# konstantineder/montecarlo-risk-engine

Measured on AMD Instinct MI355X. Metric: path-steps/sec at 1M paths x 250 steps; PV/CVA rel-error vs CPU ref, higher is better.
Workload: dtype f64

## Files before the change

montecarlo-risk-engine_amd/csrc/kf_common.h:

```cpp
#pragma once
#include <cstddef>
#include "mcx_device.h"



struct FAtom {
    int32_t reg, pad;
    double a, d, b, c0, c1;
};
struct FTerm { double w; FAtom atom; };
struct FEvent {
    int32_t kind, flags;
    int32_t term_begin, term_end;
    int32_t coeff_off, row;
    int32_t ns, sidx;
    int32_t init_state, pad;
    double strike, sign;
    double aux[4];
    FAtom num, x;
};
struct FMetricOp {
    int32_t ns, m;
    int32_t rec_profile;
    int32_t has_cva;
    double threshold;
    FAtom surv, cond;
};

struct ChunkHeader { int32_t n_ev, n_mop, n_terms, bytes; };

struct FastDate {
    int32_t valid, flags;
    int32_t ni_reg, lin_reg, n_exp, x_reg, coeff_off0, coeff_off1, rec_profile, s_reg, c_reg, pad;
    int32_t t_reg[4];
    double x_a, x_d;
    double c_a, c_b, c_c0, c_c1;
    double m_b, m_c0, m_n1, m_s1;
    double ni_c0, ni_c1;
    double k0, k1;
    double t_w[4], t_c0[4], t_c1[4];
    double thr;
    double s_b, s_c0, s_c1;
    int32_t ex_n, ex_term_off, ex_coeff_off, ex_x_reg, ex_lin_reg, ex_pad;
    double ex_k0, ex_k1, ex_strike, ex_sign, ex_x_a, ex_x_d;
    double op_strike, op_sign;
    double ex_p_lo, ex_p_hi, ex_p_ms, ex_p_ih;
    int32_t ex_p_off, ex_p_blk, ex_p_reg, ex_p_pad;
};
struct FastDateHot {
    int32_t valid, flags;
    int32_t ni_reg, lin_reg, n_exp, x_reg, coeff_off0, coeff_off1, rec_profile, s_reg, c_reg, pad;
    int32_t t_reg[4];
    double x_a, x_d;
    double c_a, c_b, c_c0, c_c1;
    double m_b, m_c0, m_n1, m_s1;
};
static_assert(sizeof(FastDateHot) == 144 && offsetof(FastDate, ni_c0) == sizeof(FastDateHot), "FastDateHot must mirror the head of FastDate");
struct LeanTerm { double w, c0, c1; int32_t reg, pad; };

struct FusedArgs {
    K1Args k1;
    const FastDate* __restrict__ fast;
    const LeanTerm* __restrict__ lterms;
    const double* __restrict__ vcoef;
    const unsigned char* __restrict__ prog;
    const int32_t* __restrict__ date_off;
    const int32_t* __restrict__ date_row;
    const double* __restrict__ coeffs;
    double* __restrict__ cfs;
    double* __restrict__ expo;
    double* __restrict__ partials;
    int64_t ld_out;
    int32_t n_dates, n_basis, n_ns, n_rec, n_expo_rows, n_stateful, chunk_cap, pad;
    int32_t rec_pv[MCX_FUSED_MAX_NS];
    int32_t rec_cva[MCX_FUSED_MAX_NS];
    double lgd[MCX_FUSED_MAX_NS];
    int32_t init_state[MCX_FUSED_MAX_STATEFUL];
};

__device__ __forceinline__ void chan_merge(double& N, double& mean, double& M2, double n, double m, double q)
{
    if (n <= 0.0) return;
    if (N == 0.0) { N = n; mean = m; M2 = q; return; }
    const double delta = m - mean, tot = N + n;
    mean += delta * n / tot;
    M2 += q + delta * delta * N * n / tot;
    N = tot;
}

#define RFL(x) __builtin_amdgcn_readfirstlane(x)

template <int NREG>
__device__ __forceinline__ double f_atom(const FAtom& a, const double (&reg)[NREG])
{
    const int r = RFL(a.reg), fl = RFL(a.pad);
    const double x = r >= 0 ? reg[r] : 0.0;
    double v = (fl & 2) ? fma(a.d, x, a.a) : 0.0;
    if (fl & 1) v = fma(a.b, mcx_exp(fma(a.c1, x, a.c0)), v);
    return v;
}

__device__ __forceinline__ double f_poly_uniform(const double* __restrict__ coeffs, int off_vgpr, int K, double x)
{
    const double* __restrict__ c = coeffs + __builtin_amdgcn_readfirstlane(off_vgpr);
    double v = 0.0, xp = 1.0;
#pragma unroll 1
    for (int k = 0; k < K; ++k) { v = fma(ldk(c + k), xp, v); xp *= x; }
    return v;
}

__device__ __forceinline__ double f_poly(const double* __restrict__ c, int K, double x)
{
    double v = 0.0, xp = 1.0;
#pragma unroll 1
    for (int k = 0; k < K; ++k) { v = fma(c[k], xp, v); xp *= x; }
    return v;
}

__device__ __forceinline__ void f_record(double v, bool live, int rec, int n_rec, bool first_tile, double* __restrict__ lds)
{
    if (first_tile) {
        __syncthreads();
        if (threadIdx.x == 0) lds[rec] = v;
        __syncthreads();
    }
    const double c = lds[rec];
    const double d = live ? v - c : 0.0;
    const double s1 = wave_sum(d), s2 = wave_sum(d * d);
    if ((threadIdx.x & 63) == 0) {
        double* acc = lds + n_rec + ((threadIdx.x >> 6) * n_rec + rec) * 2;
        acc[0] += s1;
        acc[1] += s2;
    }
}

template <int NREG>
__device__ __forceinline__ double f_regsel(int r, const double (&reg)[NREG])
{
    return r >= 0 ? reg[r] : 0.0;
}


int mcx_launch_kf_lean(const FusedArgs& a, const mcx_sim_desc& sd, int n_cu, bool inject, bool simulate, hipStream_t s);
```

montecarlo-risk-engine_amd/csrc/kf_fused.hip:

```cpp
#include "kf_common.h"

#include <algorithm>
#include <type_traits>
#include <cmath>
#include <cstdlib>

namespace {

template <int NSLOT, int SIG, int NNS, bool STORE, bool ALL_FAST>
__device__ __forceinline__ bool kf_fast_date(const FusedArgs& a, int t, int64_t i, bool live, bool first_tile, double* __restrict__ lds,
                                             const double (&reg)[2 * NSLOT], double (&cfs)[NNS], double (&cva)[NNS])
{
    constexpr int NREG = 2 * NSLOT;
    if (NNS != 1) return false;
    if (!ALL_FAST && ldk(&a.fast[t].valid) != 1) return false;
    const FastDate* __restrict__ fp = a.fast + t;
#define FD(x) ldk(&fp->x)
    const K1Args& k = a.k1;
    if (STORE && k.paths && live) sim_store_state<NSLOT, SIG>(k, t, i, reg);
    const int flags = FD(flags);
    const double inv = (flags & 16) ? FD(ni_c0) : mcx_exp(fma(FD(ni_c1), f_regsel<NREG>(FD(ni_reg), reg), FD(ni_c0)));
    if (flags & 1) {
        double val = fma(FD(k1), f_regsel<NREG>(FD(lin_reg), reg), FD(k0));
        const int n_exp = FD(n_exp);
// ... 271 lines not shown
                on_date(t, std::integral_constant<bool, false>());
                next_t = t + 1;
            }
        }
        (void)next_t;
        for (int w = 0; w < a.n_ns; ++w) {
            double cv = cfs[0], cc = cva[0];
#pragma unroll
            for (int q = 1; q < NNS; ++q) { cv = (w == q) ? cfs[q] : cv; cc = (w == q) ? cva[q] : cc; }
            if (a.cfs && live) a.cfs[(int64_t)w * a.ld_out + i] = cv;
            if (a.rec_pv[w] >= 0) f_record(cv, live, a.rec_pv[w], n_rec, first_tile, lds);
            if (a.rec_cva[w] >= 0) f_record(cc * a.lgd[w], live, a.rec_cva[w], n_rec, first_tile, lds);
        }
    }
    __syncthreads();
    for (int r = threadIdx.x; r < n_rec; r += MCX_BLOCK) {
        double s1 = 0.0, s2 = 0.0;
        for (int w = 0; w < 4; ++w) { s1 += lds[n_rec + (w * n_rec + r) * 2]; s2 += lds[n_rec + (w * n_rec + r) * 2 + 1]; }
        double* dst = a.partials + ((int64_t)blockIdx.x * n_rec + r) * 4;
        dst[0] = n_block; dst[1] = lds[r]; dst[2] = s1; dst[3] = s2;
    }
}

template <int NSLOT, int NZ, bool INJECT, int SIG, int NNS, int NST, int NPF, bool SIMULATE>
__global__ __launch_bounds__(MCX_BLOCK) void kf_fused(const FusedArgs a)
{
    kf_body<NSLOT, NZ, INJECT, SIG, NNS, NST, NPF, SIMULATE>(a);
}

__global__ __launch_bounds__(MCX_BLOCK) void kf_merge(const double* __restrict__ partials, int n_rec, int n_blocks, mcx_acc* __restrict__ out)
{
    const int r = blockIdx.x;
    __shared__ double sN[MCX_BLOCK], sM[MCX_BLOCK], sQ[MCX_BLOCK];
    double N = 0.0, mean = 0.0, M2 = 0.0;
    for (int b = threadIdx.x; b < n_blocks; b += MCX_BLOCK) {
        const double* p = partials + ((int64_t)b * n_rec + r) * 4;
        const double n = p[0];
        if (n > 0.0) chan_merge(N, mean, M2, n, p[1] + p[2] / n, fmax(p[3] - p[2] * p[2] / n, 0.0));
    }
    sN[threadIdx.x] = N; sM[threadIdx.x] = mean; sQ[threadIdx.x] = M2;
    __syncthreads();
    for (int stride = MCX_BLOCK / 2; stride > 0; stride >>= 1) {
        if ((int)threadIdx.x < stride) {
            double a = sN[threadIdx.x], b = sM[threadIdx.x], c = sQ[threadIdx.x];
            chan_merge(a, b, c, sN[threadIdx.x + stride], sM[threadIdx.x + stride], sQ[threadIdx.x + stride]);
            sN[threadIdx.x] = a; sM[threadIdx.x] = b; sQ[threadIdx.x] = c;
        }
        __syncthreads();
    }
    if (threadIdx.x == 0) { out[r].n = sN[0]; out[r].shift = sM[0]; out[r].s1 = 0.0; out[r].s2 = sQ[0]; }
}

template <int NSLOT, int NZ, int SIG>
void launch_kf(const FusedArgs& a, int grid, size_t lds, int npf, bool inject, bool simulate, hipStream_t s)
{
    const bool one_ns = a.n_ns == 1, no_state = a.n_stateful == 0;
#define MCX_KF(INJ, NNS, NST, NPF) do { if (simulate) hipLaunchKernelGGL((kf_fused<NSLOT, NZ, INJ, SIG, NNS, NST, NPF, true>), dim3(grid), dim3(MCX_BLOCK), lds, s, a); \
        else if (!INJ) hipLaunchKernelGGL((kf_fused<NSLOT, NZ, false, SIG, NNS, NST, NPF, false>), dim3(grid), dim3(MCX_BLOCK), lds, s, a); } while (0)
#define MCX_KF_NPF(INJ, NNS, NST) do { if (npf == 1) MCX_KF(INJ, NNS, NST, 1); else if (npf == 2) MCX_KF(INJ, NNS, NST, 2); else MCX_KF(INJ, NNS, NST, 0); } while (0)
    if (inject) {
        if (one_ns && no_state) MCX_KF_NPF(true, 1, 0);
        else MCX_KF(true, MCX_FUSED_MAX_NS, MCX_FUSED_MAX_STATEFUL, 0);
    } else {
        if (one_ns && no_state) MCX_KF_NPF(false, 1, 0);
        else if (one_ns) MCX_KF_NPF(false, 1, MCX_FUSED_MAX_STATEFUL);
        else MCX_KF(false, MCX_FUSED_MAX_NS, MCX_FUSED_MAX_STATEFUL, 0);
    }
#undef MCX_KF_NPF
#undef MCX_KF
}

}

struct mcx_fused {
    const mcx_sim* sim;
    const mcx_book* book;
    int n_rec, n_ns, n_dates, n_expo_rows, n_stateful, want_pv;
    unsigned char* d_prog;
    FastDate* d_fast;
    int32_t* d_date_off;
    int32_t* d_date_row;
    int chunk_cap, npf;
    int lean;
    LeanTerm* d_lterms;
    double* d_vcoef;
    int32_t rec_pv[MCX_FUSED_MAX_NS], rec_cva[MCX_FUSED_MAX_NS];
    double lgd[MCX_FUSED_MAX_NS];
    int32_t init_state[MCX_FUSED_MAX_STATEFUL];
    double* d_partials;
    size_t partial_bytes;
    mcx_acc* d_out;
    mutable hipEvent_t tev[2 * MCX_FUSED_TIMING_RING];
    mutable int timing, t_count, t_launch;
};

static void fused_timing_off(mcx_fused* f)
{
    if (f->timing) for (int q = 0; q < 2 * MCX_FUSED_TIMING_RING; ++q) hipEventDestroy(f->tev[q]);
    f->timing = 0; f->t_count = 0; f->t_launch = 0;
}

extern "C" int mcx_fused_set_timing(mcx_fused* f, int32_t enable)
{
    if (!f) return -1;
    fused_timing_off(f);
    if (enable) {
        for (int q = 0; q < 2 * MCX_FUSED_TIMING_RING; ++q)
            if (hipEventCreate(&f->tev[q]) != hipSuccess) { for (int r = 0; r < q; ++r) hipEventDestroy(f->tev[r]); return -100; }
        f->timing = enable > 0 ? enable : 1;
    }
    return 0;
}

extern "C" int mcx_fused_kernel_times(mcx_fused* f, float* h_ms, int32_t capacity, int32_t* n_out)
{
    if (!f || !h_ms || !n_out) return -1;
    *n_out = 0;
    if (!f->timing) return 0;
    const int n = f->t_count < capacity ? f->t_count : capacity;
    for (int q = 0; q < n; ++q) {
        if (hipEventSynchronize(f->tev[2 * q + 1]) != hipSuccess) return -100;
        if (hipEventElapsedTime(&h_ms[q], f->tev[2 * q], f->tev[2 * q + 1]) != hipSuccess) return -100;
    }
    *n_out = n;
    f->t_count = 0; f->t_launch = 0;
    return 0;
}

extern "C" void mcx_fused_destroy(mcx_fused* f)
{
    if (!f) return;
    fused_timing_off(f);
    hipFree(f->d_lterms); hipFree(f->d_vcoef); hipFree(f->d_prog); hipFree(f->d_fast); hipFree(f->d_date_off); hipFree(f->d_date_row); hipFree(f->d_partials); hipFree(f->d_out);
    delete f;
}

extern "C" int mcx_fused_num_records(const mcx_fused* f) { return f ? f->n_rec : -1; }

extern "C" int mcx_fused_create(mcx_handle* h, const mcx_sim* sim, const mcx_book* book, const mcx_fused_desc* d, mcx_fused** out)
{
    if (!h || !sim || !book || !d || !out) return -1;
    const mcx_sim_desc& sd = sim->desc;
    if (book->n_state != sd.n_state) MCX_FAIL(h, -2, "mcx_fused_create: book and sim disagree on the state dimension");
    if (d->n_netting_sets < 1 || d->n_netting_sets > MCX_FUSED_MAX_NS || d->n_netting_sets != book->n_netting_sets)
        MCX_FAIL(h, MCX_E_NOT_FUSABLE, "not fusable: %d netting sets (max %d)", book->n_netting_sets, MCX_FUSED_MAX_NS);
    if (d->n_expo_rows != book->n_expo_rows) MCX_FAIL(h, -2, "mcx_fused_create: n_expo_rows mismatch");
    const int T = sd.n_dates;
    for (int s = 0; s < sd.n_slots; ++s)
        if (sd.slots[s].kind == MCX_MODEL_S2F) MCX_FAIL(h, MCX_E_NOT_FUSABLE, "not fusable: the Schwartz two-factor spot is a derived state column");
    int col_reg[MCX_MAX_STATE];
    for (int s = 0; s < sd.n_slots; ++s) {
        col_reg[sd.slots[s].state_off] = 2 * s;
        if (sd.slots[s].kind != MCX_MODEL_BS) col_reg[sd.slots[s].state_off + 1] = 2 * s + 1;
    }
    bool ok = true;
    std::string why;
    auto fatom = [&](const mcx_atom& q, int t_event) {
        FAtom o; o.a = q.a; o.d = q.d; o.b = q.b; o.c0 = q.c0; o.c1 = q.c1; o.reg = -1;
        o.pad = (q.b != 0.0 ? 1 : 0) | ((q.a != 0.0 || q.d != 0.0) ? 2 : 0);
        if (q.col >= 0) {
            if (q.t_idx != t_event) { ok = false; why = "an event reads the state of another date (unequal swap tenors)"; }
            o.reg = col_reg[q.col];
        }
        return o;
    };
    const DevEventVec& hev = book->h_events;
    const std::vector<DevTerm>& hte = book->h_terms;
    auto devatom_to_mcx = [](const DevAtom& q) { mcx_atom o; o.t_idx = q.t_idx; o.col = q.col; o.a = q.a; o.d = q.d; o.b = q.b; o.c0 = q.c0; o.c1 = q.c1; return o; };

    std::vector<std::vector<FEvent>> by_date(T);
    std::vector<std::vector<int>> by_date_q(T);
    std::vector<std::vector<FTerm>> terms_by_date(T);
    int n_stateful = 0;
    int32_t init_state[MCX_FUSED_MAX_STATEFUL] = {0, 0, 0, 0};
    if ((int)book->h_event_t_idx.size() != book->n_events) MCX_FAIL(h, -2, "mcx_fused_create: internal (event dates missing)");
    for (int p = 0; p < book->n_products && ok; ++p) {
        const DevProduct& pr = book->h_products[p];
        if (pr.ev_end == pr.ev_begin) continue;
        int sidx = -1;
        if (pr.n_states > 1) {
            if (n_stateful >= MCX_FUSED_MAX_STATEFUL) { ok = false; why = "too many exercise products"; break; }
            sidx = n_stateful;
            init_state[n_stateful++] = pr.init_state;
        }
        for (int q = pr.ev_begin; q < pr.ev_end && ok; ++q) {
            const DevEvent& e = hev[q];
            const int t = book->h_event_t_idx[q];
            if (t < 0 || t >= T) { ok = false; why = "event date out of range"; break; }
            FEvent fe;
            memset(&fe, 0, sizeof(fe));
            fe.kind = e.kind; fe.flags = e.flags; fe.coeff_off = e.coeff_off; fe.row = e.row; fe.ns = pr.netting_set; fe.sidx = sidx;
            fe.init_state = pr.init_state; fe.pad = pr.n_states; fe.strike = e.strike; fe.sign = e.sign;
            for (int w = 0; w < 4; ++w) fe.aux[w] = e.aux[w];
            if (e.kind == MCX_EV_OPTION && (e.aux[0] == 4.0 || e.aux[0] == 5.0)) { ok = false; why = "barrier monitoring is evaluated by the book kernel (K2)"; }
            fe.num = fatom(devatom_to_mcx(e.num), t);
            fe.x = fatom(devatom_to_mcx(e.x), t);
            std::vector<FTerm>& terms = terms_by_date[t];
            fe.term_begin = (int)terms.size();
            for (int j = e.term_begin; j < e.term_end; ++j) {
                if (hte[j].den >= 0) { ok = false; why = "a cashflow term carries its own numeraire (unequal swap tenors)"; break; }
                FTerm ft; ft.w = hte[j].w; ft.atom = fatom(devatom_to_mcx(hte[j].atom), t);
                terms.push_back(ft);
            }
            fe.term_end = (int)terms.size();
            if (!by_date[t].empty() && memcmp(&by_date[t].back().num, &fe.num, sizeof(FAtom)) == 0) fe.flags |= 2;
            else fe.flags &= ~2;
            by_date[t].push_back(fe);
            by_date_q[t].push_back(q);
        }
    }
    std::vector<std::vector<FMetricOp>> mop_by_date(T);
    std::vector<int32_t> date_row(T, -1);
    for (int r = 0; r < d->n_expo_rows; ++r) {
        const int t = d->row_t_idx[r];
        if (t < 0 || t >= T) MCX_FAIL(h, -2, "mcx_fused_create: exposure row %d has no timeline date", r);
        date_row[t] = r;
// ... 102 lines not shown
                    if (tm.atom.b != 0.0) {
                        if (fd.n_exp >= 4) { okf = false; break; }
                        fd.t_reg[fd.n_exp] = tm.atom.reg; fd.t_w[fd.n_exp] = tm.w * tm.atom.b;
                        fd.t_c0[fd.n_exp] = tm.atom.c0; fd.t_c1[fd.n_exp] = tm.atom.c1; fd.n_exp++;
                    }
                }
            } else {
                if (e.x.b != 0.0 || n_expo >= 2) { okf = false; break; }
                if ((fd.flags & 2) && (fd.x_reg != e.x.reg || fd.x_a != e.x.a || fd.x_d != e.x.d)) { okf = false; break; }
                if (stateful && n_expo > 0) { okf = false; break; }
                if ((fd.flags & 256)) { okf = false; break; }
                fd.flags |= 2; fd.x_reg = e.x.reg; fd.x_a = e.x.a; fd.x_d = e.x.d;
                int off = e.coeff_off >= 0 ? e.coeff_off + e.init_state * book->n_basis : -1;
                if (stateful) { fd.flags |= 256; lean_only = true; off = e.coeff_off; if (off < 0) { okf = false; break; } }
                (n_expo == 0 ? fd.coeff_off0 : fd.coeff_off1) = off;
                n_expo++;
            }
        }
        if (okf && num) {
            if (num->a == 0.0 && num->d == 0.0 && num->b > 0.0) { fd.ni_reg = num->reg; fd.ni_c0 = -num->c0 - log(num->b); fd.ni_c1 = -num->c1; }
            else if (num->b == 0.0 && num->d == 0.0 && num->a != 0.0) { fd.flags |= 16; fd.ni_c0 = 1.0 / num->a; }
            else okf = false;
        }
        if (okf && mop_by_date[t].size() > 1) okf = false;
        if (okf && mop_by_date[t].size() == 1) {
            const FMetricOp& mo = mop_by_date[t][0];
            fd.flags |= 32; fd.thr = mo.threshold;
            if (mo.rec_profile >= 0) { fd.flags |= 8; fd.rec_profile = mo.rec_profile; }
            if (mo.has_cva) {
                if (mo.surv.a != 0.0 || mo.surv.d != 0.0 || mo.cond.d != 0.0) okf = false;
                fd.flags |= 4;
                fd.s_reg = mo.surv.reg; fd.s_b = mo.surv.b; fd.s_c0 = mo.surv.c0; fd.s_c1 = mo.surv.c1;
                fd.c_reg = mo.cond.reg; fd.c_a = mo.cond.a; fd.c_b = mo.cond.b; fd.c_c0 = mo.cond.c0; fd.c_c1 = mo.cond.c1;
            }
        }
        if (okf && !num && !mop_by_date[t].empty()) { fd.flags |= 16; fd.ni_c0 = 1.0; }
        auto bind = [](int32_t& r, double& coef) { if (r < 0) { r = 0; coef = 0.0; } };
        bind(fd.ni_reg, fd.ni_c1); bind(fd.lin_reg, fd.k1); bind(fd.x_reg, fd.x_d); bind(fd.s_reg, fd.s_c1); bind(fd.c_reg, fd.c_c1);
        bind(fd.ex_x_reg, fd.ex_x_d); bind(fd.ex_lin_reg, fd.ex_k1);
        for (int j = 0; j < 4; ++j) bind(fd.t_reg[j], fd.t_c1[j]);
        if (okf && (fd.flags & 4) && !(fd.flags & 8) && fd.thr == 0.0) {
            fd.flags |= 64;
            if (fd.flags & 16) { fd.m_b = fd.s_b * fd.ni_c0; fd.m_c0 = fd.s_c0; fd.m_n1 = 0.0; }
            else { fd.m_b = fd.s_b; fd.m_c0 = fd.s_c0 + fd.ni_c0; fd.m_n1 = fd.ni_c1; }
            fd.m_s1 = fd.s_c1;
        }
        if (!okf) lterms.resize(fd.ex_term_off <= (int32_t)lterms.size() && (fd.flags & 128) ? fd.ex_term_off : lterms.size());
        fd.valid = okf ? (lean_only ? 2 : 1) : 0;
        fast[t] = fd;
    }
    std::vector<unsigned char> prog;
    std::vector<int32_t> date_off(T + 1, 0);
    int max_chunk = 0;
    bool bs_exposure = false;
    for (int t = 0; t < T; ++t) for (const FEvent& e : by_date[t]) if (e.kind == MCX_EV_EXPO_BS) bs_exposure = true;
    for (int t = 0; t < T; ++t) {
        date_off[t] = (int32_t)prog.size();
        if (fast[t].valid == 1) continue;
        ChunkHeader hd;
        hd.n_ev = (int)by_date[t].size(); hd.n_mop = (int)mop_by_date[t].size(); hd.n_terms = (int)terms_by_date[t].size();
        const size_t bytes = sizeof(hd) + sizeof(FEvent) * by_date[t].size() + sizeof(FTerm) * terms_by_date[t].size() +
                             sizeof(FMetricOp) * mop_by_date[t].size();
        const size_t padded = (bytes + 15) & ~(size_t)15;
        hd.bytes = (int32_t)padded;
        const size_t base = prog.size();
        prog.resize(base + padded, 0);
        unsigned char* p = prog.data() + base;
        memcpy(p, &hd, sizeof(hd)); p += sizeof(hd);
        if (hd.n_ev) { memcpy(p, by_date[t].data(), sizeof(FEvent) * by_date[t].size()); p += sizeof(FEvent) * by_date[t].size(); }
        if (hd.n_terms) { memcpy(p, terms_by_date[t].data(), sizeof(FTerm) * terms_by_date[t].size()); p += sizeof(FTerm) * terms_by_date[t].size(); }
        if (hd.n_mop) memcpy(p, mop_by_date[t].data(), sizeof(FMetricOp) * mop_by_date[t].size());
        max_chunk = std::max(max_chunk, (int)padded);
    }
    date_off[T] = (int32_t)prog.size();
    if (bs_exposure) { delete f; MCX_FAIL(h, MCX_E_NOT_FUSABLE, "not fusable: analytic Black-Scholes exposures are evaluated by the book kernel (K2)"); }
    bool all_fast = d->n_netting_sets == 1 && n_stateful == 0, lean = d->n_netting_sets == 1 && n_stateful <= 1;
    for (int t = 0; t < T; ++t) { all_fast = all_fast && fast[t].valid == 1; lean = lean && fast[t].valid != 0; }
    f->npf = max_chunk <= 1024 ? 1 : (max_chunk <= 2048 ? 2 : 0);
    f->chunk_cap = f->npf > 0 ? f->npf * 1024 : ((max_chunk + 255) & ~255);
    if (all_fast) { f->npf = -1; f->chunk_cap = 0; }
    for (int q = 0; q < sd.n_slots; ++q)
        if (sd.slots[q].kind == MCX_MODEL_CIRPP && !(sd.init_state[sd.slots[q].state_off] > 0.0)) lean = false;
    f->lean = lean ? 1 : 0;
    if ((size_t)4 * f->chunk_cap + sizeof(double) * 9 * (size_t)n_rec > 60 * 1024) {
        delete f;
        MCX_FAIL(h, MCX_E_NOT_FUSABLE, "not fusable: a date's event program (%d B) exceeds the per-wave LDS slot budget", max_chunk);
    }

    f->sim = sim; f->book = book; f->n_rec = n_rec; f->n_ns = d->n_netting_sets; f->n_dates = T; f->n_expo_rows = d->n_expo_rows;
    f->n_stateful = n_stateful; f->want_pv = d->want_pv;
    for (int q = 0; q < MCX_FUSED_MAX_STATEFUL; ++q) f->init_state[q] = init_state[q];
    auto up = [&](void** dst, const void* src, size_t bytes) -> hipError_t {
        hipError_t e = hipMalloc(dst, bytes ? bytes : 8);
        if (e != hipSuccess) return e;
        return bytes ? hipMemcpy(*dst, src, bytes, hipMemcpyHostToDevice) : hipSuccess;
    };
    prog.resize(prog.size() + 4096, 0);
    lterms.resize(lterms.size() + 1);
    vcoef.resize(vcoef.size() + MCX_VPOLY_BLK, 0.0);
    f->partial_bytes = sizeof(double) * 4 * (size_t)n_rec * 2048;
    hipError_t e = up((void**)&f->d_prog, prog.data(), prog.size());
    if (e == hipSuccess) e = up((void**)&f->d_fast, fast.data(), sizeof(FastDate) * fast.size());
    if (e == hipSuccess) e = up((void**)&f->d_lterms, lterms.data(), sizeof(LeanTerm) * lterms.size());
    if (e == hipSuccess) e = up((void**)&f->d_vcoef, vcoef.data(), sizeof(double) * vcoef.size());
    if (e == hipSuccess) e = up((void**)&f->d_date_off, date_off.data(), sizeof(int32_t) * date_off.size());
    if (e == hipSuccess) e = up((void**)&f->d_date_row, date_row.data(), sizeof(int32_t) * date_row.size());
    if (e == hipSuccess) e = hipMalloc(&f->d_partials, f->partial_bytes);
    if (e == hipSuccess) e = hipMalloc(&f->d_out, sizeof(mcx_acc) * (size_t)n_rec);
    if (e != hipSuccess) {
        mcx_fused_destroy(f);
        MCX_FAIL(h, -100 - (int)e, "mcx_fused_create: %s", hipGetErrorString(e));
    }
    *out = f;
    return 0;
}

static int fused_run_impl(mcx_handle* h, const mcx_fused* f, bool simulate, uint64_t seed, uint64_t path_offset, int64_t n_paths,
                          double* d_paths, int64_t ld, double* d_cfs, double* d_expo, int64_t ld_out,
                          const double* d_inject_z, const double* d_inject_u, mcx_acc* h_out, mcx_acc* d_out, void* stream)
{
    if (!h || !f || (h_out == nullptr) == (d_out == nullptr)) return -1;
    if (n_paths <= 0) {
        if (h_out) memset(h_out, 0, sizeof(mcx_acc) * (size_t)f->n_rec);
        else MCX_HIP(h, hipMemsetAsync(d_out, 0, sizeof(mcx_acc) * (size_t)f->n_rec, (hipStream_t)stream));
        return 0;
    }
    if ((d_paths || d_inject_z) && ld < n_paths) MCX_FAIL(h, -2, "mcx_fused_run: ld < n_paths");
    if ((d_cfs || d_expo) && ld_out < n_paths) MCX_FAIL(h, -2, "mcx_fused_run: ld_out < n_paths");
    if ((size_t)f->n_rec * sizeof(mcx_acc) > h->pinned_bytes) MCX_FAIL(h, -2, "mcx_fused_run: too many records");
    const mcx_sim_desc& sd = f->sim->desc;
    if (sd.n_uniform && d_inject_z && !d_inject_u) MCX_FAIL(h, -3, "mcx_fused_run: inject_u required with inject_z under QE");
    if (!simulate && (!d_paths || ld < n_paths)) MCX_FAIL(h, -2, "mcx_fused_eval_paths: a paths tensor with ld >= n_paths is required");
    FusedArgs a;
    memset(&a, 0, sizeof(a));
    mcx_fill_k1_args(f->sim, seed, path_offset, n_paths, ld > 0 ? ld : n_paths, d_paths, d_inject_z, d_inject_u, &a.k1);
    a.prog = f->d_prog; a.fast = f->d_fast; a.lterms = f->d_lterms; a.vcoef = f->d_vcoef; a.date_off = f->d_date_off; a.chunk_cap = f->chunk_cap;
    a.date_row = f->d_date_row; a.coeffs = f->book->d_coeffs; a.cfs = d_cfs; a.expo = d_expo; a.partials = f->d_partials;
    a.ld_out = ld_out; a.n_dates = f->n_dates; a.n_basis = f->book->n_basis; a.n_ns = f->n_ns; a.n_rec = f->n_rec;
    a.n_expo_rows = f->n_expo_rows; a.n_stateful = f->n_stateful;
    for (int k = 0; k < MCX_FUSED_MAX_NS; ++k) { a.rec_pv[k] = f->rec_pv[k]; a.rec_cva[k] = f->rec_cva[k]; a.lgd[k] = f->lgd[k]; }
    for (int k = 0; k < MCX_FUSED_MAX_STATEFUL; ++k) a.init_state[k] = f->init_state[k];
    hipStream_t s = (hipStream_t)stream;
    const bool inj = d_inject_z != nullptr;
    int grid;
    const bool timed = f->timing && (f->t_launch++ % f->timing) == 0 && f->t_count < MCX_FUSED_TIMING_RING;
    if (timed) MCX_HIP(h, hipEventRecord(f->tev[2 * f->t_count], s));
    const bool direct = !d_out && sizeof(mcx_acc) * (size_t)f->n_rec <= h->pinned_bytes && h->d_pinned_alias;
    mcx_acc* dst = d_out ? d_out : (direct ? (mcx_acc*)h->d_pinned_alias : f->d_out);
    if (f->lean && (simulate || !inj)) {
        grid = mcx_launch_kf_lean(a, sd, h->n_cu, inj, simulate, s);
        if (grid < 0) MCX_FAIL(h, MCX_E_NOT_FUSABLE, "not fusable: (slots=%d, z=%d) has no fused instantiation", sd.n_slots, sd.n_z);
    } else {
        const int64_t tiles = (n_paths + MCX_BLOCK - 1) / MCX_BLOCK;
        grid = (int)std::min<int64_t>(tiles, 2048);
        if (tiles > 2048) { int per = (int)((tiles + 2047) / 2048); grid = (int)((tiles + per - 1) / per); }
        const size_t lds = sizeof(double) * (size_t)((9 * f->n_rec + 1) & ~1) + (size_t)4 * f->chunk_cap;
        switch (mcx_sim_signature(sd)) {
        case SIG_VAS_CIR_E: launch_kf<2, 2, SIG_VAS_CIR_E>(a, grid, lds, f->npf, inj, simulate, s); break;
        case SIG_BS_A: launch_kf<1, 1, SIG_BS_A>(a, grid, lds, f->npf, inj, simulate, s); break;
        case SIG_BS_E: launch_kf<1, 1, SIG_BS_E>(a, grid, lds, f->npf, inj, simulate, s); break;
        case SIG_HESTON_QE: launch_kf<1, 2, SIG_HESTON_QE>(a, grid, lds, f->npf, inj, simulate, s); break;
        case SIG_HESTON_E: launch_kf<1, 2, SIG_HESTON_E>(a, grid, lds, f->npf, inj, simulate, s); break;
        case SIG_VAS_E: launch_kf<1, 1, SIG_VAS_E>(a, grid, lds, f->npf, inj, simulate, s); break;
        case SIG_VAS_A: launch_kf<1, 1, SIG_VAS_A>(a, grid, lds, f->npf, inj, simulate, s); break;
        case SIG_BS_VAS_CIRDET_E: launch_kf<3, 3, SIG_BS_VAS_CIRDET_E>(a, grid, lds, f->npf, inj, simulate, s); break;
        default:
            switch (sd.n_slots * 16 + sd.n_z) {
            case 1 * 16 + 1: launch_kf<1, 1, SIG_GENERIC>(a, grid, lds, f->npf, inj, simulate, s); break;
            case 1 * 16 + 2: launch_kf<1, 2, SIG_GENERIC>(a, grid, lds, f->npf, inj, simulate, s); break;
            case 2 * 16 + 2: launch_kf<2, 2, SIG_GENERIC>(a, grid, lds, f->npf, inj, simulate, s); break;
            case 3 * 16 + 3: launch_kf<3, 3, SIG_GENERIC>(a, grid, lds, f->npf, inj, simulate, s); break;
            case 4 * 16 + 4: launch_kf<4, 4, SIG_GENERIC>(a, grid, lds, f->npf, inj, simulate, s); break;
            default: MCX_FAIL(h, MCX_E_NOT_FUSABLE, "not fusable: (slots=%d, z=%d) has no fused instantiation", sd.n_slots, sd.n_z);
            }
        }
    }
    MCX_HIP(h, hipGetLastError());
    if (timed) { MCX_HIP(h, hipEventRecord(f->tev[2 * f->t_count + 1], s)); ++f->t_count; }
    hipLaunchKernelGGL(kf_merge, dim3(f->n_rec), dim3(MCX_BLOCK), 0, s, f->d_partials, f->n_rec, grid, dst);
    MCX_HIP(h, hipGetLastError());
    if (d_out) return 0;
    if (!direct) MCX_HIP(h, hipMemcpyAsync(h->h_pinned, f->d_out, sizeof(mcx_acc) * (size_t)f->n_rec, hipMemcpyDeviceToHost, s));
    MCX_HIP(h, hipStreamSynchronize(s));
    memcpy(h_out, h->h_pinned, sizeof(mcx_acc) * (size_t)f->n_rec);
    return 0;
}

extern "C" int mcx_fused_is_straight_line(const mcx_fused* f)
{
    return (f && f->lean) ? 1 : 0;
}

extern "C" int mcx_fused_run(mcx_handle* h, const mcx_fused* f, uint64_t seed, uint64_t path_offset, int64_t n_paths,
                             double* d_paths, int64_t ld, double* d_cfs, double* d_expo, int64_t ld_out,
                             const double* d_inject_z, const double* d_inject_u, mcx_acc* h_out, void* stream)
{
    return fused_run_impl(h, f, true, seed, path_offset, n_paths, d_paths, ld, d_cfs, d_expo, ld_out, d_inject_z, d_inject_u, h_out, nullptr, stream);
}

extern "C" int mcx_fused_run_device(mcx_handle* h, const mcx_fused* f, uint64_t seed, uint64_t path_offset, int64_t n_paths,
                                    double* d_paths, int64_t ld, double* d_cfs, double* d_expo, int64_t ld_out,
                                    const double* d_inject_z, const double* d_inject_u, mcx_acc* d_out, void* stream)
{
    return fused_run_impl(h, f, true, seed, path_offset, n_paths, d_paths, ld, d_cfs, d_expo, ld_out, d_inject_z, d_inject_u, nullptr, d_out, stream);
}

extern "C" int mcx_fused_eval_paths(mcx_handle* h, const mcx_fused* f, const double* d_paths, int64_t n_paths, int64_t ld,
                                    double* d_cfs, double* d_expo, int64_t ld_out, mcx_acc* h_out, void* stream)
{
    return fused_run_impl(h, f, false, 0, 0, n_paths, const_cast<double*>(d_paths), ld, d_cfs, d_expo, ld_out, nullptr, nullptr, h_out, nullptr, stream);
}

extern "C" int mcx_fused_eval_paths_device(mcx_handle* h, const mcx_fused* f, const double* d_paths, int64_t n_paths, int64_t ld,
                                           double* d_cfs, double* d_expo, int64_t ld_out, mcx_acc* d_out, void* stream)
{
    return fused_run_impl(h, f, false, 0, 0, n_paths, const_cast<double*>(d_paths), ld, d_cfs, d_expo, ld_out, nullptr, nullptr, nullptr, d_out, stream);
}
```

montecarlo-risk-engine_amd/csrc/kf_lean.hip:

```cpp
#include <cstdlib>
#include <map>
#include <utility>

#include "kf_common.h"

namespace {

#define FD(x) ldk(&fp->x)

typedef const MCX_KONST FusedArgs KArgs;
__device__ __forceinline__ KArgs& kargs_region(int z)
{
    return *(KArgs*)((const MCX_KONST char*)__builtin_amdgcn_kernarg_segment_ptr() + z);
}

template <int PPL>
__device__ __forceinline__ void lean_poly_add(const double* __restrict__ c, int K, const double (&x)[PPL], double (&p)[PPL])
{
    if (K == 3) {
        const double c0 = ldk(c), c1 = ldk(c + 1), c2 = ldk(c + 2);
#pragma unroll
        for (int q = 0; q < PPL; ++q) p[q] += fma(fma(c2, x[q], c1), x[q], c0);
    } else {
        double v[PPL];
// ... 181 lines not shown
            est[q] = ex ? est[q] - 1 : est[q];
        }
    }
    double p[PPL];
#pragma unroll
    for (int q = 0; q < PPL; ++q) p[q] = 0.0;
    if (flags & 2) {
        const double xa = FD(x_a), xd = FD(x_d);
        const int xr = FD(x_reg), off0 = FD(coeff_off0), off1 = FD(coeff_off1);
        double x[PPL];
#pragma unroll
        for (int q = 0; q < PPL; ++q) x[q] = fma(xd, reg[q][xr], xa);
        if (flags & 256) {
            double p0[PPL], p1[PPL];
#pragma unroll
            for (int q = 0; q < PPL; ++q) { p0[q] = 0.0; p1[q] = 0.0; }
            lean_poly_add<PPL>(a.coeffs + off0, a.n_basis, x, p0);
            lean_poly_add<PPL>(a.coeffs + off0 + a.n_basis, a.n_basis, x, p1);
#pragma unroll
            for (int q = 0; q < PPL; ++q) p[q] = est[q] > 0 ? p1[q] : p0[q];
        } else {
            if (off0 >= 0) lean_poly_add<PPL>(a.coeffs + off0, a.n_basis, x, p);
            if (off1 >= 0) lean_poly_add<PPL>(a.coeffs + off1, a.n_basis, x, p);
        }
    }
    auto cond_surv = [&](double (&cs)[PPL]) {
        const double ca = FD(c_a), cb = FD(c_b);
#pragma unroll
        for (int q = 0; q < PPL; ++q) cs[q] = ca;
        if (cb != 0.0) {
            const double cc0 = FD(c_c0), cc1 = FD(c_c1);
            const int cr = FD(c_reg);
#pragma unroll
            for (int q = 0; q < PPL; ++q) cs[q] = fma(cb, mcx_exp_tab(fma(cc1, reg[q][cr], cc0), etab, ec), ca);
        }
    };
    if (merged) {
        const double mb = FD(m_b), mc0 = FD(m_c0), mn1 = FD(m_n1), ms1 = FD(m_s1);
        const int nr = FD(ni_reg), sr = FD(s_reg);
        double w[PPL], cs[PPL];
#pragma unroll
        for (int q = 0; q < PPL; ++q) w[q] = mb * mcx_exp_tab(fma(ms1, reg[q][sr], fma(mn1, reg[q][nr], mc0)), etab, ec);
        cond_surv(cs);
#pragma unroll
        for (int q = 0; q < PPL; ++q) cva[q] = fma(fmax(p[q], 0.0), w[q] * (1.0 - cs[q]), cva[q]);
        return;
    }
    double e[PPL];
#pragma unroll
    for (int q = 0; q < PPL; ++q) e[q] = p[q] * inv[q];
    if (a.expo) {
        const int row = ldk(a.date_row + t);
        if (row >= 0) {
#pragma unroll
            for (int q = 0; q < PPL; ++q) if (live[q]) a.expo[(int64_t)row * a.ld_out + i[q]] = e[q];
        }
    }
    if (flags & 32) {
        const double thr = FD(thr);
        double u[PPL];
#pragma unroll
        for (int q = 0; q < PPL; ++q) u[q] = dev_thr(e[q], thr);
        if (flags & 8) {
            const int rp = FD(rec_profile);
            double up[PPL], un[PPL];
#pragma unroll
            for (int q = 0; q < PPL; ++q) { up[q] = fmax(u[q], 0.0); un[q] = fmin(u[q], 0.0); }
            lean_record<PPL>(up, live, rp, a.n_rec, first_tile, lds);
            lean_record<PPL>(un, live, rp + 1, a.n_rec, first_tile, lds);
        }
        if (flags & 4) {
            const double sb = FD(s_b), sc0 = FD(s_c0), sc1 = FD(s_c1);
            const int sr = FD(s_reg);
            double sp[PPL], cs[PPL];
#pragma unroll
            for (int q = 0; q < PPL; ++q) sp[q] = sb * mcx_exp_tab(fma(sc1, reg[q][sr], sc0), etab, ec);
            cond_surv(cs);
#pragma unroll
            for (int q = 0; q < PPL; ++q) cva[q] = fma(fmax(u[q], 0.0), sp[q] * (1.0 - cs[q]), cva[q]);
        }
    }
}

#define MCX_LEAN_WAVES 4
template <int NSLOT, int NZ, bool INJECT, int SIG, int PPL, bool SIMULATE>
__global__ __launch_bounds__(MCX_BLOCK, MCX_LEAN_WAVES) void kf_lean(const FusedArgs)
{
    constexpr int NREG = 2 * NSLOT;
    constexpr int TILE = MCX_BLOCK * PPL;
    extern __shared__ double lds[];
    KArgs& a0 = kargs_region(0);
    const int n_rec = a0.n_rec;
    const int64_t n = a0.k1.n;
    for (int q = threadIdx.x; q < 9 * n_rec; q += MCX_BLOCK) lds[q] = 0.0;
    constexpr int BMB = SIG == SIG_VAS_CIR_E ? 10 : 7;
    constexpr int BM = (INJECT || !SIMULATE) ? 0 : MCX_BM_LDS_DOUBLES_B(BMB);
    __shared__ double tab_lds[BM + MCX_EXP_LDS_DOUBLES];
    const double* tab = nullptr;
    const double* etab = tab_lds + BM;
    mcx_exp_tab_load(tab_lds + BM);
    if (BM) { mcx_bm_load<BMB>(tab_lds); tab = tab_lds; }
    __syncthreads();
    const int64_t tiles = (n + TILE - 1) / TILE;
    double n_block = 0.0;

    for (int64_t tile = blockIdx.x; tile < tiles; tile += gridDim.x) {
        const bool first_tile = tile == (int64_t)blockIdx.x;
        int64_t i[PPL];
        bool live[PPL];
        uint64_t path[PPL];
        double reg[PPL][NREG];
        double cfs[PPL], cva[PPL];
        int est[PPL];
        int n_init, n_steps;
        {
            KArgs& a = kargs_region(mcx_region_zero());
            const auto& k = a.k1;
#pragma unroll
            for (int q = 0; q < PPL; ++q) {
                const int64_t i_raw = tile * TILE + q * MCX_BLOCK + threadIdx.x;
                live[q] = i_raw < n;
                i[q] = live[q] ? i_raw : n - 1;
                path[q] = k.path_offset + (uint64_t)i[q];
                sim_init_state<NSLOT, SIG>(k, reg[q]);
                cfs[q] = 0.0; cva[q] = 0.0;
                est[q] = a.init_state[0];
            }
            const int64_t rest = n - tile * TILE;
            n_block += (double)(rest < TILE ? rest : TILE);
            n_init = k.n_initial_store; n_steps = k.n_steps;
        }
        if (SIMULATE) {
        int step = 0, t_init = 0;
#pragma unroll 1
        while (true) {
            const bool init = t_init < n_init;
            if (!init && step >= n_steps) break;
            int st = init ? t_init : -1;
            t_init += init ? 1 : 0;
            {
                const int zr0 = mcx_region_zero();
                const auto& k = kargs_region(zr0).k1;
                const uint64_t seed = k.seed;
                const mcx_bm_coef bc = mcx_bm_coef_load(zr0);
                const mcx_bm_vconst vc = mcx_bm_vconst_make<BMB>(bc);
#pragma unroll 1
                while (st < 0 && step < n_steps) {
                    if constexpr (SIG == SIG_GENERIC) {
#pragma unroll
                        for (int q = 0; q < PPL; ++q) sim_substep<NSLOT, NZ, INJECT, SIG, BMB, true>(k, step, path[q], i[q], reg[q], tab, seed, bc, &vc);
                        st = ldk(&k.steps[step].store_idx);
                    } else {
                        double zz[PPL][NZ], uu[PPL];
                        bool rare = false;
                        const StepData<NSLOT, NZ> sdat = sim_step_load<NSLOT, NZ, SIG>(k, step);
                        __builtin_amdgcn_sched_barrier(0);
                        if constexpr (INJECT) {
#pragma unroll
                            for (int q = 0; q < PPL; ++q) sim_draw<NZ, true, SIG, BMB>(k, step, path[q], i[q], zz[q], uu[q], tab, seed, bc, &vc);
                        } else {
                            uint32_t st_q[PPL];
#pragma unroll
                            for (int q = 0; q < PPL; ++q) st_q[q] = (uint32_t)step;
                            rare = sim_draw_n<PPL, NZ, SIG, BMB>(k, st_q, path, zz, uu, tab, seed, bc, vc);
                        }
                        if (!INJECT && __builtin_expect(__any(rare), 0)) {
#pragma unroll
                            for (int q = 0; q < PPL; ++q) sim_draw<NZ, false, SIG, BMB, true>(k, step, path[q], i[q], zz[q], uu[q], tab, seed, bc, &vc);
                        }
#pragma unroll
                        for (int q = 0; q < PPL; ++q) st = sim_apply_loaded<NSLOT, NZ, SIG, true>(k, sdat, reg[q], zz[q], uu[q]);
                    }
                    ++step;
                }
            }
            if (st >= 0) lean_date<NSLOT, SIG, PPL, true>(st, i, live, first_tile, lds, reg, cfs, cva, est, etab);
        }
        } else {
            auto load_row = [&](int t, double (&dst)[PPL][NREG]) {
                const auto& k = kargs_region(0).k1;
                const int D = k.n_state;
#pragma unroll
                for (int q = 0; q < PPL; ++q)
#pragma unroll
                    for (int sl = 0; sl < NSLOT; ++sl) {
                        const bool bs = sig_kind(SIG, sl) >= 0 ? sig_is_bs(SIG, sl) : (k.slots[sl].kind == MCX_MODEL_BS);
                        const int c = k.slots[sl].state_off;
                        dst[q][2 * sl] = k.paths[((int64_t)t * D + c) * k.ld + i[q]];
                        dst[q][2 * sl + 1] = bs ? 0.0 : k.paths[((int64_t)t * D + c + 1) * k.ld + i[q]];
                    }
            };
            const int n_dates = kargs_region(0).n_dates;
            double bufb[PPL][NREG];
            load_row(0, reg);
            load_row(n_dates > 1 ? 1 : 0, bufb);
#pragma unroll 1
            for (int t = 0; t < n_dates; t += 2) {
                lean_date<NSLOT, SIG, PPL, false>(t, i, live, first_tile, lds, reg, cfs, cva, est, etab);
                if (t + 2 < n_dates) load_row(t + 2, reg);
                if (t + 1 < n_dates) {
                    lean_date<NSLOT, SIG, PPL, false>(t + 1, i, live, first_tile, lds, bufb, cfs, cva, est, etab);
                    if (t + 3 < n_dates) load_row(t + 3, bufb);
                }
            }
        }
        {
            KArgs& a = kargs_region(mcx_region_zero());
#pragma unroll
            for (int q = 0; q < PPL; ++q) if (a.cfs && live[q]) a.cfs[i[q]] = cfs[q];
            if (a.rec_pv[0] >= 0) lean_record<PPL>(cfs, live, a.rec_pv[0], n_rec, first_tile, lds);
            if (a.rec_cva[0] >= 0) {
                const double lgd = a.lgd[0];
                double cc[PPL];
#pragma unroll
                for (int q = 0; q < PPL; ++q) cc[q] = cva[q] * lgd;
                lean_record<PPL>(cc, live, a.rec_cva[0], n_rec, first_tile, lds);
            }
        }
    }
    __syncthreads();
    for (int r = threadIdx.x; r < n_rec; r += MCX_BLOCK) {
        double s1 = 0.0, s2 = 0.0;
        for (int w = 0; w < 4; ++w) { s1 += lds[n_rec + (w * n_rec + r) * 2]; s2 += lds[n_rec + (w * n_rec + r) * 2 + 1]; }
        double* dst = a0.partials + ((int64_t)blockIdx.x * n_rec + r) * 4;
        dst[0] = n_block; dst[1] = lds[r]; dst[2] = s1; dst[3] = s2;
    }
}

#undef FD

template <int NSLOT, int NZ, int SIG, int PPL>
int launch_lean_shape(const FusedArgs& a, int n_cu, bool inject, bool simulate, hipStream_t s)
{
    const int64_t tiles = (a.k1.n + MCX_BLOCK * PPL - 1) / (MCX_BLOCK * PPL);
    const size_t lds = sizeof(double) * (size_t)((9 * a.n_rec + 1) & ~1);
    auto residency = [&](auto kernel) {
        thread_local std::map<std::pair<const void*, size_t>, int> cache;
        const auto key = std::make_pair((const void*)kernel, lds);
        auto it = cache.find(key);
        if (it == cache.end()) {
            int per_cu = 0;
            if (hipOccupancyMaxActiveBlocksPerMultiprocessor(&per_cu, kernel, MCX_BLOCK, lds) != hipSuccess || per_cu < 1) per_cu = 1;
            it = cache.emplace(key, per_cu < MCX_LEAN_WAVES ? per_cu : MCX_LEAN_WAVES).first;
        }
        return (int64_t)it->second * n_cu;
    };
    auto sized = [&](int64_t resident) {
        if (tiles <= resident) return (int)tiles;
        const int64_t per = (tiles + resident - 1) / resident;
        return (int)((tiles + per - 1) / per);
    };
    int grid;
    if (!simulate) {
        auto kern = kf_lean<NSLOT, NZ, false, SIG, PPL, false>;
        grid = sized(residency(kern));
        hipLaunchKernelGGL(kern, dim3(grid), dim3(MCX_BLOCK), lds, s, a);
    } else if (inject) {
        auto kern = kf_lean<NSLOT, NZ, true, SIG, PPL, true>;
        grid = sized(residency(kern));
        hipLaunchKernelGGL(kern, dim3(grid), dim3(MCX_BLOCK), lds, s, a);
    } else {
        auto kern = kf_lean<NSLOT, NZ, false, SIG, PPL, true>;
        grid = sized(residency(kern));
        hipLaunchKernelGGL(kern, dim3(grid), dim3(MCX_BLOCK), lds, s, a);
    }
    return grid;
}

template <int NSLOT, int NZ, int SIG>
void launch_lean(const FusedArgs& a, int n_cu, bool inject, bool simulate, hipStream_t s, int* grid_out)
{
    constexpr int PPL = (SIG == SIG_GENERIC && NSLOT >= 2) ? 1 : 2;
#ifdef MCX_LEAN_AB
    if (simulate && !inject) {
        const char* sh = getenv("MCX_LEAN_SHAPE");
        const int code = sh ? atoi(sh) : 0;
        if (code == 11) { *grid_out = launch_lean_shape<NSLOT, NZ, SIG, 1>(a, n_cu, inject, simulate, s); return; }
        if (code == 21) { *grid_out = launch_lean_shape<NSLOT, NZ, SIG, 2>(a, n_cu, inject, simulate, s); return; }
    }
#endif
    const int64_t full_tiles = (a.k1.n + MCX_BLOCK * PPL - 1) / (MCX_BLOCK * PPL);
    if (PPL == 2 && simulate && !inject && full_tiles < (int64_t)2 * n_cu) {
        *grid_out = launch_lean_shape<NSLOT, NZ, SIG, 1>(a, n_cu, inject, simulate, s);
        return;
    }
    *grid_out = launch_lean_shape<NSLOT, NZ, SIG, PPL>(a, n_cu, inject, simulate, s);
}

}

int mcx_launch_kf_lean(const FusedArgs& a, const mcx_sim_desc& sd, int n_cu, bool inject, bool simulate, hipStream_t s)
{
    int grid = -1;
    switch (mcx_sim_signature(sd)) {
    case SIG_VAS_CIR_E: launch_lean<2, 2, SIG_VAS_CIR_E>(a, n_cu, inject, simulate, s, &grid); break;
#ifndef MCX_LEAN_ONE_SIG
    case SIG_BS_A: launch_lean<1, 1, SIG_BS_A>(a, n_cu, inject, simulate, s, &grid); break;
    case SIG_BS_E: launch_lean<1, 1, SIG_BS_E>(a, n_cu, inject, simulate, s, &grid); break;
    case SIG_HESTON_QE: launch_lean<1, 2, SIG_HESTON_QE>(a, n_cu, inject, simulate, s, &grid); break;
    case SIG_HESTON_E: launch_lean<1, 2, SIG_HESTON_E>(a, n_cu, inject, simulate, s, &grid); break;
    case SIG_VAS_E: launch_lean<1, 1, SIG_VAS_E>(a, n_cu, inject, simulate, s, &grid); break;
    case SIG_VAS_A: launch_lean<1, 1, SIG_VAS_A>(a, n_cu, inject, simulate, s, &grid); break;
    case SIG_BS_VAS_CIRDET_E: launch_lean<3, 3, SIG_BS_VAS_CIRDET_E>(a, n_cu, inject, simulate, s, &grid); break;
    default:
        switch (sd.n_slots * 16 + sd.n_z) {
        case 1 * 16 + 1: launch_lean<1, 1, SIG_GENERIC>(a, n_cu, inject, simulate, s, &grid); break;
        case 1 * 16 + 2: launch_lean<1, 2, SIG_GENERIC>(a, n_cu, inject, simulate, s, &grid); break;
        case 2 * 16 + 2: launch_lean<2, 2, SIG_GENERIC>(a, n_cu, inject, simulate, s, &grid); break;
        case 3 * 16 + 3: launch_lean<3, 3, SIG_GENERIC>(a, n_cu, inject, simulate, s, &grid); break;
        case 4 * 16 + 4: launch_lean<4, 4, SIG_GENERIC>(a, n_cu, inject, simulate, s, &grid); break;
        default: break;
        }
#else
    default: break;
#endif
    }
    return grid;
}
```

Before: 270.3 billion.

## Add specialized CVA-only date kernel with per-date params and regression coefficients in LDS

Adds a compact per-date CVA parameter table, built on the host when the book is CVA-only with the Vasicek+CIR++ signature and three basis functions. It also adds a kernel variant that stages these parameters and the regression coefficient rows into LDS at block start. Each exposure date then runs a branch-free routine that evaluates two polynomial rows, batches its exponentials through the table exp, and accumulates CVA. This drops the generic per-date flag decoding and scattered global constant loads. The cost is more LDS per block, so the path is used only when occupancy stays unchanged and only for plain simulate runs with no outputs requested.

Measured after the change: 291.6 billion (median of 6 runs). 7.9% higher.

```diff
diff --git a/montecarlo-risk-engine_amd/csrc/kf_common.h b/montecarlo-risk-engine_amd/csrc/kf_common.h
--- a/montecarlo-risk-engine_amd/csrc/kf_common.h
+++ b/montecarlo-risk-engine_amd/csrc/kf_common.h
@@ -58,9 +58,25 @@
 static_assert(sizeof(FastDateHot) == 144 && offsetof(FastDate, ni_c0) == sizeof(FastDateHot), "FastDateHot must mirror the head of FastDate");
 struct LeanTerm { double w, c0, c1; int32_t reg, pad; };
 
+struct alignas(16) FastDateCva {
+    double m_s1, m_n1, m_c0, m_b;
+    double c_c1, c_c0, c_a, c_b;
+    double x_d, x_a;
+    int32_t coeff_off0, coeff_off1, pad[2];
+};
+struct alignas(16) FastDateCvaLds {
+    double m_s1, m_n1, m_c0, m_b, c_c1, c_c0, c_a, c_b, x_d, x_a;
+    double row0[3], row1[3];
+};
+#define FDC_HEAD 10
+static_assert(sizeof(FastDateCva) == 96 && offsetof(FastDateCva, coeff_off0) == FDC_HEAD * sizeof(double), "FastDateCva layout");
+static_assert(sizeof(FastDateCvaLds) == 128 && offsetof(FastDateCvaLds, row0) == FDC_HEAD * sizeof(double), "FastDateCvaLds layout");
+enum { FDC_X_REG = 0, FDC_NI_REG = 1, FDC_C_REG = 2, FDC_S_REG = 3 };
+
 struct FusedArgs {
     K1Args k1;
     const FastDate* __restrict__ fast;
+    const FastDateCva* __restrict__ cva_dates;
     const LeanTerm* __restrict__ lterms;
     const double* __restrict__ vcoef;
     const unsigned char* __restrict__ prog;
diff --git a/montecarlo-risk-engine_amd/csrc/kf_fused.hip b/montecarlo-risk-engine_amd/csrc/kf_fused.hip
--- a/montecarlo-risk-engine_amd/csrc/kf_fused.hip
+++ b/montecarlo-risk-engine_amd/csrc/kf_fused.hip
@@ -377,6 +377,7 @@
     int32_t* d_date_row;
     int chunk_cap, npf;
     int lean;
+    FastDateCva* d_cva;
     LeanTerm* d_lterms;
     double* d_vcoef;
     int32_t rec_pv[MCX_FUSED_MAX_NS], rec_cva[MCX_FUSED_MAX_NS];
@@ -426,7 +427,7 @@
 {
     if (!f) return;
     fused_timing_off(f);
-    hipFree(f->d_lterms); hipFree(f->d_vcoef); hipFree(f->d_prog); hipFree(f->d_fast); hipFree(f->d_date_off); hipFree(f->d_date_row); hipFree(f->d_partials); hipFree(f->d_out);
+    hipFree(f->d_lterms); hipFree(f->d_vcoef); hipFree(f->d_cva); hipFree(f->d_prog); hipFree(f->d_fast); hipFree(f->d_date_off); hipFree(f->d_date_row); hipFree(f->d_partials); hipFree(f->d_out);
     delete f;
 }
 
@@ -695,6 +696,23 @@
     for (int q = 0; q < sd.n_slots; ++q)
         if (sd.slots[q].kind == MCX_MODEL_CIRPP && !(sd.init_state[sd.slots[q].state_off] > 0.0)) lean = false;
     f->lean = lean ? 1 : 0;
+    std::vector<FastDateCva> cva_dates(T);
+    bool cva_only = lean && mcx_sim_signature(sd) == SIG_VAS_CIR_E && f->rec_pv[0] < 0 && f->rec_cva[0] >= 0 && book->n_basis == 3;
+    for (int t = 0; t < T && cva_only; ++t) {
+        const FastDate& fd = fast[t];
+        FastDateCva& c = cva_dates[t];
+        memset(&c, 0, sizeof(c));
+        c.coeff_off0 = c.coeff_off1 = -1;
+        if ((fd.flags & (64 | 128 | 256)) == 64) {
+            cva_only = fd.c_b != 0.0 && fd.s_reg == FDC_S_REG && fd.ni_reg == FDC_NI_REG && fd.c_reg == FDC_C_REG && fd.x_reg == FDC_X_REG;
+            c.m_s1 = fd.m_s1; c.m_n1 = fd.m_n1; c.m_c0 = fd.m_c0; c.m_b = fd.m_b;
+            c.c_c1 = fd.c_c1; c.c_c0 = fd.c_c0; c.c_a = fd.c_a; c.c_b = fd.c_b;
+            c.x_d = fd.x_d; c.x_a = fd.x_a;
+            if (fd.flags & 2) { c.coeff_off0 = fd.coeff_off0; c.coeff_off1 = fd.coeff_off1; }
+        } else if (fd.flags & (32 | 128 | 256)) {
+            cva_only = false;
+        }
+    }
     if ((size_t)4 * f->chunk_cap + sizeof(double) * 9 * (size_t)n_rec > 60 * 1024) {
         delete f;
         MCX_FAIL(h, MCX_E_NOT_FUSABLE, "not fusable: a date's event program (%d B) exceeds the per-wave LDS slot budget", max_chunk);
@@ -714,6 +732,7 @@
     f->partial_bytes = sizeof(double) * 4 * (size_t)n_rec * 2048;
     hipError_t e = up((void**)&f->d_prog, prog.data(), prog.size());
     if (e == hipSuccess) e = up((void**)&f->d_fast, fast.data(), sizeof(FastDate) * fast.size());
+    if (e == hipSuccess && cva_only) e = up((void**)&f->d_cva, cva_dates.data(), sizeof(FastDateCva) * cva_dates.size());
     if (e == hipSuccess) e = up((void**)&f->d_lterms, lterms.data(), sizeof(LeanTerm) * lterms.size());
     if (e == hipSuccess) e = up((void**)&f->d_vcoef, vcoef.data(), sizeof(double) * vcoef.size());
     if (e == hipSuccess) e = up((void**)&f->d_date_off, date_off.data(), sizeof(int32_t) * date_off.size());
@@ -747,6 +766,7 @@
     FusedArgs a;
     memset(&a, 0, sizeof(a));
     mcx_fill_k1_args(f->sim, seed, path_offset, n_paths, ld > 0 ? ld : n_paths, d_paths, d_inject_z, d_inject_u, &a.k1);
+    a.cva_dates = (simulate && !d_inject_z && !d_paths && !d_cfs && !d_expo) ? f->d_cva : nullptr;
     a.prog = f->d_prog; a.fast = f->d_fast; a.lterms = f->d_lterms; a.vcoef = f->d_vcoef; a.date_off = f->d_date_off; a.chunk_cap = f->chunk_cap;
     a.date_row = f->d_date_row; a.coeffs = f->book->d_coeffs; a.cfs = d_cfs; a.expo = d_expo; a.partials = f->d_partials;
     a.ld_out = ld_out; a.n_dates = f->n_dates; a.n_basis = f->book->n_basis; a.n_ns = f->n_ns; a.n_rec = f->n_rec;
diff --git a/montecarlo-risk-engine_amd/csrc/kf_lean.hip b/montecarlo-risk-engine_amd/csrc/kf_lean.hip
--- a/montecarlo-risk-engine_amd/csrc/kf_lean.hip
+++ b/montecarlo-risk-engine_amd/csrc/kf_lean.hip
@@ -287,10 +287,36 @@
     }
 }
 
+template <int NSLOT, int PPL>
+__device__ __forceinline__ void lean_date_cva(const FastDateCvaLds* __restrict__ rp, const double (&reg)[PPL][2 * NSLOT], double (&cva)[PPL],
+                                              const double* __restrict__ etab)
+{
+    const mcx_expq_coef ec = mcx_expq_load(mcx_region_zero());
+    const FastDateCvaLds r = *rp;
+    double xe[2 * PPL], ev[2 * PPL];
+#pragma unroll
+    for (int q = 0; q < PPL; ++q) {
+        xe[2 * q] = fma(r.m_s1, reg[q][FDC_S_REG], fma(r.m_n1, reg[q][FDC_NI_REG], r.m_c0));
+        xe[2 * q + 1] = fma(r.c_c1, reg[q][FDC_C_REG], r.c_c0);
+    }
+    mcx_exp_tab_n<2 * PPL>(xe, ev, etab, ec);
+#pragma unroll
+    for (int q = 0; q < PPL; ++q) {
+        const double x = fma(r.x_d, reg[q][FDC_X_REG], r.x_a);
+        double p = 0.0;
+        p += fma(fma(r.row0[2], x, r.row0[1]), x, r.row0[0]);
+        p += fma(fma(r.row1[2], x, r.row1[1]), x, r.row1[0]);
+        const double w = r.m_b * ev[2 * q];
+        const double cs = fma(r.c_b, ev[2 * q + 1], r.c_a);
+        cva[q] = fma(fmax(p, 0.0), w * (1.0 - cs), cva[q]);
+    }
+}
+
 #define MCX_LEAN_WAVES 4
-template <int NSLOT, int NZ, bool INJECT, int SIG, int PPL, bool SIMULATE>
+template <int NSLOT, int NZ, bool INJECT, int SIG, int PPL, bool SIMULATE, int DK = 0>
 __global__ __launch_bounds__(MCX_BLOCK, MCX_LEAN_WAVES) void kf_lean(const FusedArgs)
 {
+    static_assert(DK == 0 || (SIG == SIG_VAS_CIR_E && SIMULATE && !INJECT), "the cva-date kernel simulates the Vasicek + CIR++ signature");
     constexpr int NREG = 2 * NSLOT;
     constexpr int TILE = MCX_BLOCK * PPL;
     extern __shared__ double lds[];
@@ -298,6 +324,23 @@
     const int n_rec = a0.n_rec;
     const int64_t n = a0.k1.n;
     for (int q = threadIdx.x; q < 9 * n_rec; q += MCX_BLOCK) lds[q] = 0.0;
+    FastDateCvaLds* const dlds = (FastDateCvaLds*)(lds + ((9 * n_rec + 1) & ~1));
+    if constexpr (DK == 1) {
+        const FastDateCva* __restrict__ dc = a0.cva_dates;
+        const double* __restrict__ cf = a0.coeffs;
+        const int n_dates = a0.n_dates;
+        for (int q = threadIdx.x; q < 16 * n_dates; q += MCX_BLOCK) {
+            const int t = q >> 4, e = q & 15;
+            double v;
+            if (e < FDC_HEAD) {
+                v = ((const double*)(dc + t))[e];
+            } else {
+                const int off = e < FDC_HEAD + 3 ? dc[t].coeff_off0 : dc[t].coeff_off1;
+                v = off >= 0 ? cf[off + (e - FDC_HEAD) % 3] : 0.0;
+            }
+            ((double*)dlds)[q] = v;
+        }
+    }
     constexpr int BMB = SIG == SIG_VAS_CIR_E ? 10 : 7;
     constexpr int BM = (INJECT || !SIMULATE) ? 0 : MCX_BM_LDS_DOUBLES_B(BMB);
     __shared__ double tab_lds[BM + MCX_EXP_LDS_DOUBLES];
@@ -379,7 +422,10 @@
                     ++step;
                 }
             }
-            if (st >= 0) lean_date<NSLOT, SIG, PPL, true>(st, i, live, first_tile, lds, reg, cfs, cva, est, etab);
+            if (st >= 0) {
+                if constexpr (DK == 1) lean_date_cva<NSLOT, PPL>(dlds + st, reg, cva, etab);
+                else lean_date<NSLOT, SIG, PPL, true>(st, i, live, first_tile, lds, reg, cfs, cva, est, etab);
+            }
         }
         } else {
             auto load_row = [&](int t, double (&dst)[PPL][NREG]) {
@@ -439,13 +485,14 @@
 {
     const int64_t tiles = (a.k1.n + MCX_BLOCK * PPL - 1) / (MCX_BLOCK * PPL);
     const size_t lds = sizeof(double) * (size_t)((9 * a.n_rec + 1) & ~1);
-    auto residency = [&](auto kernel) {
+    const size_t lds_cva = lds + sizeof(FastDateCvaLds) * (size_t)a.n_dates;
+    auto residency = [&](auto kernel, size_t bytes) {
         thread_local std::map<std::pair<const void*, size_t>, int> cache;
-        const auto key = std::make_pair((const void*)kernel, lds);
+        const auto key = std::make_pair((const void*)kernel, bytes);
         auto it = cache.find(key);
         if (it == cache.end()) {
             int per_cu = 0;
-            if (hipOccupancyMaxActiveBlocksPerMultiprocessor(&per_cu, kernel, MCX_BLOCK, lds) != hipSuccess || per_cu < 1) per_cu = 1;
+            if (hipOccupancyMaxActiveBlocksPerMultiprocessor(&per_cu, kernel, MCX_BLOCK, bytes) != hipSuccess || per_cu < 1) per_cu = 1;
             it = cache.emplace(key, per_cu < MCX_LEAN_WAVES ? per_cu : MCX_LEAN_WAVES).first;
         }
         return (int64_t)it->second * n_cu;
@@ -458,15 +505,24 @@
     int grid;
     if (!simulate) {
         auto kern = kf_lean<NSLOT, NZ, false, SIG, PPL, false>;
-        grid = sized(residency(kern));
+        grid = sized(residency(kern, lds));
         hipLaunchKernelGGL(kern, dim3(grid), dim3(MCX_BLOCK), lds, s, a);
     } else if (inject) {
         auto kern = kf_lean<NSLOT, NZ, true, SIG, PPL, true>;
-        grid = sized(residency(kern));
+        grid = sized(residency(kern, lds));
         hipLaunchKernelGGL(kern, dim3(grid), dim3(MCX_BLOCK), lds, s, a);
     } else {
         auto kern = kf_lean<NSLOT, NZ, false, SIG, PPL, true>;
-        grid = sized(residency(kern));
+        const int64_t resident = residency(kern, lds);
+        if constexpr (SIG == SIG_VAS_CIR_E) {
+            auto kern_cva = kf_lean<NSLOT, NZ, false, SIG, PPL, true, 1>;
+            if (a.cva_dates && residency(kern_cva, lds_cva) >= resident) {
+                grid = sized(resident);
+                hipLaunchKernelGGL(kern_cva, dim3(grid), dim3(MCX_BLOCK), lds_cva, s, a);
+                return grid;
+            }
+        }
+        grid = sized(resident);
         hipLaunchKernelGGL(kern, dim3(grid), dim3(MCX_BLOCK), lds, s, a);
     }
     return grid;
```
